# graphdeco-inria/hierarchical-3d-gaussians

Hardware: NVIDIA B200
Metric: train-step images/sec (fwd+bwd) @1080p, 3M Gaussians, SH-3 (higher is better)
Workload: dtype f32

## Files before the change

hierarchical-3d-gaussians_b200/csrc/common.cuh:

```cuda
#pragma once
#include <cuda_runtime.h>
#include <stdint.h>
#include <stdio.h>
#include <stdlib.h>
#include "../../include/h3dgs.h"

namespace h3dgs {

constexpr float kNearPlane = 0.2f;
constexpr float kFovClamp = 1.3f;
constexpr float kDilation = 0.3f;
constexpr float kLambdaFloor = 0.1f;
constexpr int kTile = H3DGS_TILE;
constexpr int kTilePixels = kTile * kTile;
constexpr float kAlphaCap = 0.99f;
constexpr float kAlphaSkip = 1.0f / 255.0f;
constexpr float kTStop = 0.0001f;
constexpr float kWEps = 0.0000001f;
constexpr uint32_t kKidsMask = 0xFFFFFu;
constexpr int kClampShift = 20;
constexpr uint32_t kSortedKidsMask = 0xFFFu;
constexpr int kBlockShift = 16;

struct __align__(16) Record { float4 a, b, c; };
static_assert(sizeof(Record) == 48, "record must be 48 bytes");

__host__ __device__ inline size_t align_up(size_t x, size_t a = 256) { return (x + a - 1) / a * a; }

struct GeomLayout {
    size_t depths, tiles_touched, offsets, rank_mask, records, scan_temp, total;
    size_t scan_temp_bytes;
};
struct BinLayout {
    size_t keys_unsorted, keys_sorted, vals_unsorted, vals_sorted, sort_temp, sorted_records, total;
    size_t sort_temp_bytes;
};
struct ImgLayout {
    size_t final_T, n_contrib, ranges, tile_max_contrib, tile_count, scan_info, total;
};
struct ScanInfo { uint32_t D, max_count, overflow, prefilter_bad; };
constexpr int kTileSortCap = 8192;

GeomLayout geom_layout(int P);
BinLayout bin_layout(int64_t D);
ImgLayout img_layout(int W, int H);

void prof_begin(int stage, cudaStream_t s);
void prof_end(int stage, cudaStream_t s);
struct ProfScope {
    int stage; cudaStream_t s;
    ProfScope(int st, cudaStream_t ss) : stage(st), s(ss) { prof_begin(stage, s); }
    ~ProfScope() { prof_end(stage, s); }
};

int pinned_scratch(void** out);

void set_error(const char* fmt, ...);
extern int64_t g_launches;

#define H3_CUDA(call)                                                                      \
    do {                                                                                   \
        cudaError_t e__ = (call);                                                          \
        if (e__ != cudaSuccess) {                                                          \
            h3dgs::set_error("%s failed at %s:%d: %s", #call, __FILE__, __LINE__,          \
                             cudaGetErrorString(e__));                                     \
            return H3DGS_ECUDA;                                                            \
        }                                                                                  \
    } while (0)

#define H3_LAUNCHED(name, debug, stream)                                                   \
    do {                                                                                   \
        h3dgs::g_launches++;                                                               \
        cudaError_t e__ = cudaGetLastError();                                              \
        if (e__ == cudaSuccess && (debug)) e__ = cudaStreamSynchronize(stream);            \
        if (e__ != cudaSuccess) {                                                          \
            h3dgs::set_error("kernel %s failed: %s", name, cudaGetErrorString(e__));       \
            return H3DGS_ECUDA;                                                            \
        }                                                                                  \
    } while (0)

int launch_preprocess(const h3dgs_raster_args& a, int32_t* radii, float* depths, uint32_t* tiles_touched,
                      uint8_t* rank_mask, Record* records, uint32_t* tile_count, ScanInfo* info, cudaStream_t s);
int launch_tile_scan(const h3dgs_raster_args& a, const uint32_t* tile_count, uint32_t* ranges, ScanInfo* info,
                     uint32_t cap_entries, uint32_t cap_list, cudaStream_t s);
int launch_tile_binning(const h3dgs_raster_args& a, const int32_t* radii, const float* depths, const Record* records,
                        int64_t D, uint32_t max_count, uint8_t* bin, const BinLayout& bl, const uint32_t* ranges,
                        const ScanInfo* info, uint32_t* tile_count, cudaStream_t s);
int launch_preprocess_color(const h3dgs_raster_args& a, const int32_t* radii, const uint32_t* tiles_touched,
                            Record* records, cudaStream_t s);
int launch_sh_backward(const h3dgs_raster_args& a, const int32_t* radii, const uint8_t* rank_mask, const Record* records,
                       const float* accum, float* dL_dmeans3D, float* dL_dsh, cudaStream_t s);
int launch_scan(const uint32_t* in, uint32_t* out, int n, void* temp, size_t temp_bytes, cudaStream_t s, bool debug);
size_t scan_temp_bytes(int n);
size_t sort_temp_bytes(int64_t n);
int launch_binning(const h3dgs_raster_args& a, const int32_t* radii, const float* depths, const uint32_t* offsets,
                   const Record* records, int64_t D, uint8_t* bin, const BinLayout& bl, uint32_t* ranges,
                   cudaStream_t s);
int launch_render_forward(const h3dgs_raster_args& a, const uint32_t* ranges, const Record* sorted_records,
                          float* out_color, float* out_invdepth, float* final_T, uint32_t* n_contrib,
                          uint32_t* tile_max_contrib, cudaStream_t s);
int launch_render_backward(const h3dgs_raster_args& a, const uint32_t* ranges, const Record* sorted_records,
                           const uint32_t* point_list, const float* final_T, const uint32_t* n_contrib,
                           const uint32_t* tile_max_contrib, const float* dL_dcolor, const float* dL_dinvdepth,
                           float* accum , cudaStream_t s);
int launch_preprocess_backward(const h3dgs_raster_args& a, const int32_t* radii, const uint8_t* rank_mask, const Record* records,
                               const float* accum, float* dL_dmeans3D, float* dL_dmeans2D, float* dL_dsh,
                               float* dL_dcolors, float* dL_dopacities, float* dL_dscales, float* dL_drots,
                               float* dL_dcov3D, cudaStream_t s);

#ifdef __CUDACC__
__device__ __forceinline__ void quad_pixel(int tile_x, int tile_y, int warp, int lane, int& px, int& py0) {
    px = tile_x * kTile + 8 * (warp & 1) + (lane & 7);
    py0 = tile_y * kTile + 8 * (warp >> 1) + 2 * (lane >> 3);
}

__device__ __forceinline__ void group_pixel(int tile_x, int tile_y, int warp, int lane, int& px, int& py0) {
    const int g = lane >> 3, k = lane & 7;
    px = tile_x * kTile + 8 * (warp & 1) + 4 * (g & 1) + (k & 3);
    py0 = tile_y * kTile + 8 * (warp >> 1) + 4 * (g >> 1) + 2 * (k >> 2);
}
inline bool use_group_walk() { const char* e = getenv("H3DGS_GROUPWALK"); return !(e && e[0] == '0'); }

#endif

struct PeerPtrs { void* p[H3DGS_MAX_PEERS]; int n; };
inline PeerPtrs peer_ptrs(void* const* src, int n) {
    PeerPtrs r; r.n = n > 1 ? n : 0;
    for (int k = 0; k < H3DGS_MAX_PEERS; k++) r.p[k] = (k < r.n) ? src[k] : nullptr;
    return r;
}
struct RowCycle { int shift, world, rank; };
inline RowCycle row_cycle(const h3dgs_raster_args& a) {
    RowCycle c; c.world = a.peer_count > 1 ? a.peer_count : 0; c.rank = a.shard_index; c.shift = a.grad_cyclic_log2;
    return c;
}
inline int cyclic_local_rows(const RowCycle& c, int P) {
    const int blocks = (P + (1 << c.shift) - 1) >> c.shift;
    return ((blocks + c.world - 1 - c.rank) / c.world) << c.shift;
}
#ifdef __CUDACC__
__device__ __forceinline__ int cyclic_row(const RowCycle& c, int local) {
    return ((((local >> c.shift) * c.world + c.rank)) << c.shift) + (local & ((1 << c.shift) - 1));
}
__device__ __forceinline__ bool cyclic_owned(const RowCycle& c, int row) { return ((row >> c.shift) % c.world) == c.rank; }
#endif

#ifdef __CUDACC__
struct StagePtrs { const float* own; const float* stage; int n, rank; size_t slot_floats; };
template <int NPAIR>
__device__ __forceinline__ void gather_accum_pairs(const StagePtrs& sp, uint32_t mask, int i, int first, float (&out)[2 * NPAIR]) {
#pragma unroll
    for (int k = 0; k < 2 * NPAIR; k++) out[k] = 0.f;
#pragma unroll
    for (int r = 0; r < H3DGS_MAX_PEERS; r++) {
        if (r < sp.n && ((mask >> r) & 1u)) {
            const float* row = (r == sp.rank ? sp.own : sp.stage + (size_t)r * sp.slot_floats) + (size_t)i * 10 + 2 * first;
#pragma unroll
            for (int k = 0; k < NPAIR; k++) {
                const float2 v = __ldcg(reinterpret_cast<const float2*>(row + 2 * k));
                out[2 * k] += v.x; out[2 * k + 1] += v.y;
            }
        }
    }
}
#endif
inline StagePtrs stage_ptrs(const h3dgs_raster_args& a, const float* accum) {
    StagePtrs sp; sp.own = accum; sp.n = a.peer_count > 1 ? a.peer_count : 0; sp.rank = a.shard_index;
    sp.stage = sp.n ? static_cast<const float*>(a.peer_stage[a.shard_index]) : nullptr;
    sp.slot_floats = (size_t)a.P * 10;
    return sp;
}
int launch_peer_push(const h3dgs_raster_args& a, const uint8_t* rank_mask, const float* accum, cudaStream_t s);

#ifdef H3_SIMT_EMU
extern long long g_emu_stats[16];
#define H3_STAT(i, n) (h3dgs::g_emu_stats[i] += (n))
#else
#define H3_STAT(i, n) ((void)0)
#endif

constexpr int kAccum = 10;

}

#ifdef __CUDACC__
#include "pair_math.cuh"
#endif
```

hierarchical-3d-gaussians_b200/csrc/pair_math.cuh:

```cuda
#pragma once

#ifdef H3_PAIR_HOST_EMU
#include <math.h>
#include <stdint.h>
#define H3_PM_FN static inline
namespace h3dgs {
#ifndef H3_SIMT_EMU
struct float4 { float x, y, z, w; };
constexpr float kAlphaCap = 0.99f;
constexpr float kAlphaSkip = 1.0f / 255.0f;
constexpr float kTStop = 0.0001f;
constexpr uint32_t kSortedKidsMask = 0xFFFu;
#endif
struct f2 { float lo, hi; };
H3_PM_FN f2 pk(float lo, float hi) { return f2{lo, hi}; }
H3_PM_FN void upk(f2 v, float& lo, float& hi) { lo = v.lo; hi = v.hi; }
H3_PM_FN f2 fma2(f2 a, f2 b, f2 c) { return f2{fmaf(a.lo, b.lo, c.lo), fmaf(a.hi, b.hi, c.hi)}; }
H3_PM_FN f2 mul2(f2 a, f2 b) { return f2{a.lo * b.lo, a.hi * b.hi}; }
H3_PM_FN f2 add2(f2 a, f2 b) { return f2{a.lo + b.lo, a.hi + b.hi}; }
H3_PM_FN f2 sub2(f2 a, f2 b) { return f2{a.lo - b.lo, a.hi - b.hi}; }
H3_PM_FN float fast_exp2(float x) { return exp2f(x); }
H3_PM_FN float fast_log2(float x) { return log2f(x); }
H3_PM_FN float rcp_approx(float x) { return 1.0f / x; }
H3_PM_FN float rsq_approx(float x) { return 1.0f / sqrtf(x); }
#else
#define H3_PM_FN __device__ __forceinline__
namespace h3dgs {
#ifdef H3_PAIR_SCALAR
struct f2 { float lo, hi; };
H3_PM_FN f2 pk(float lo, float hi) { return f2{lo, hi}; }
H3_PM_FN void upk(f2 v, float& lo, float& hi) { lo = v.lo; hi = v.hi; }
H3_PM_FN f2 fma2(f2 a, f2 b, f2 c) { return f2{__fmaf_rn(a.lo, b.lo, c.lo), __fmaf_rn(a.hi, b.hi, c.hi)}; }
H3_PM_FN f2 mul2(f2 a, f2 b) { return f2{__fmul_rn(a.lo, b.lo), __fmul_rn(a.hi, b.hi)}; }
H3_PM_FN f2 add2(f2 a, f2 b) { return f2{__fadd_rn(a.lo, b.lo), __fadd_rn(a.hi, b.hi)}; }
H3_PM_FN f2 sub2(f2 a, f2 b) { return f2{__fsub_rn(a.lo, b.lo), __fsub_rn(a.hi, b.hi)}; }
#else
typedef unsigned long long f2;
H3_PM_FN f2 pk(float lo, float hi) { f2 r; asm("mov.b64 %0, {%1, %2};" : "=l"(r) : "f"(lo), "f"(hi)); return r; }
H3_PM_FN void upk(f2 v, float& lo, float& hi) { asm("mov.b64 {%0, %1}, %2;" : "=f"(lo), "=f"(hi) : "l"(v)); }
H3_PM_FN f2 fma2(f2 a, f2 b, f2 c) { f2 d; asm("fma.rn.f32x2 %0, %1, %2, %3;" : "=l"(d) : "l"(a), "l"(b), "l"(c)); return d; }
H3_PM_FN f2 mul2(f2 a, f2 b) { f2 d; asm("mul.rn.f32x2 %0, %1, %2;" : "=l"(d) : "l"(a), "l"(b)); return d; }
H3_PM_FN f2 add2(f2 a, f2 b) { f2 d; asm("add.rn.f32x2 %0, %1, %2;" : "=l"(d) : "l"(a), "l"(b)); return d; }
H3_PM_FN f2 sub2(f2 a, f2 b) { f2 d; asm("sub.rn.f32x2 %0, %1, %2;" : "=l"(d) : "l"(a), "l"(b)); return d; }
#endif
H3_PM_FN float fast_exp2(float x) { float y; asm("ex2.approx.ftz.f32 %0, %1;" : "=f"(y) : "f"(x)); return y; }
H3_PM_FN float fast_log2(float x) { float y; asm("lg2.approx.ftz.f32 %0, %1;" : "=f"(y) : "f"(x)); return y; }
H3_PM_FN float rcp_approx(float x) { float y; asm("rcp.approx.ftz.f32 %0, %1;" : "=f"(y) : "f"(x)); return y; }
H3_PM_FN float rsq_approx(float x) { float y; asm("rsqrt.approx.ftz.f32 %0, %1;" : "=f"(y) : "f"(x)); return y; }
#endif

H3_PM_FN f2 bc(float x) { return pk(x, x); }
H3_PM_FN float lo(f2 v) { float a, b; upk(v, a, b); return a; }
H3_PM_FN float hi(f2 v) { float a, b; upk(v, a, b); return b; }
H3_PM_FN float hsum(f2 v) { float a, b; upk(v, a, b); return a + b; }
H3_PM_FN f2 sel2(bool p0, bool p1, f2 x, f2 y) {
    float x0, x1, y0, y1; upk(x, x0, x1); upk(y, y0, y1);
    return pk(p0 ? x0 : y0, p1 ? x1 : y1);
}
H3_PM_FN f2 ex2_2(f2 v) { float a, b; upk(v, a, b); return pk(fast_exp2(a), fast_exp2(b)); }
H3_PM_FN float fast_rcp(float x) { const float r = rcp_approx(x); return r * (2.0f - x * r); }
H3_PM_FN f2 rcp2(f2 x) {
    float x0, x1; upk(x, x0, x1);
    const f2 r = pk(rcp_approx(x0), rcp_approx(x1));
    return mul2(r, sub2(bc(2.0f), mul2(x, r)));
}

H3_PM_FN f2 pair_power(const float4& a, const float4& bb, float dx, f2 nfpy, f2& d) {
    d = add2(bc(a.y), nfpy);
    const float A = (a.z * dx) * (dx * -0.5f), B = -a.w * dx, C = -0.5f * bb.x;
    return fma2(fma2(bc(C), d, bc(B)), d, bc(A));
}
H3_PM_FN void pair_gauss(f2 power, float opacity, f2& G, f2& abase) {
    G = ex2_2(mul2(power, bc(1.4426950408889634f)));
    float a0, a1; upk(mul2(bc(opacity), G), a0, a1);
    abase = pk(fminf(kAlphaCap, a0), fminf(kAlphaCap, a1));
}
template <bool HIER, bool GRAD>
H3_PM_FN void pair_hier_alpha(f2 a, float t, uint32_t k , f2& alpha, f2& dadb) {
    alpha = a; dadb = bc(1.0f);
    if (!HIER) return;
    if (k <= 1u || t >= 1.0f) return;
    const float u = 1.0f - t;
    float a0, a1; upk(a, a0, a1);
    float o0, o1; upk(sub2(bc(1.0f), a), o0, o1);
    if (k == 2u) {
        const f2 r = pk(rsq_approx(o0), rsq_approx(o1));
        const f2 s = mul2(pk(o0, o1), r);
        f2 S = fma2(a, bc(0.02734375f), bc(0.0390625f));
        S = fma2(a, S, bc(0.0625f));
        S = fma2(a, S, bc(0.125f));
        S = fma2(a, S, bc(0.5f));
        const f2 omr = sel2(a0 < 0.0625f, a1 < 0.0625f, mul2(a, S), sub2(bc(1.0f), s));
        alpha = fma2(bc(u), omr, mul2(bc(t), a));
        if (GRAD) dadb = fma2(bc(0.5f * u), r, bc(t));
        return;
    }
    const float ik = fast_rcp((float)k);
    const f2 l2 = pk(fast_log2(o0), fast_log2(o1));
    f2 L = fma2(a, bc(0.2f), bc(0.25f));
    L = fma2(a, L, bc(0.33333334f));
    L = fma2(a, L, bc(0.5f));
    L = fma2(a, L, bc(1.0f));
    const f2 yn = mul2(mul2(a, L), bc(ik));
    f2 S = fma2(yn, bc(-0.041666668f), bc(0.16666667f));
    S = fma2(yn, S, bc(-0.5f));
    S = fma2(yn, S, bc(1.0f));
    const f2 omr_series = mul2(yn, S);
    const f2 omr_mufu = sub2(bc(1.0f), ex2_2(mul2(l2, bc(ik))));
    const f2 omr = sel2(a0 < 0.0625f, a1 < 0.0625f, omr_series, omr_mufu);
    alpha = fma2(bc(u), omr, mul2(bc(t), a));
    if (GRAD) dadb = fma2(bc(u * ik), ex2_2(mul2(l2, bc(ik - 1.0f))), bc(t));
}

H3_PM_FN f2 pair_blend(f2 pw, f2 al, f2& T, bool& done0, bool& done1, bool& v0, bool& v1, bool active = true) {
    const f2 tT = mul2(T, sub2(bc(1.0f), al));
    float pw0, pw1, al0, al1, tT0, tT1;
    upk(pw, pw0, pw1); upk(al, al0, al1); upk(tT, tT0, tT1);
    v0 = active && !done0 && pw0 <= 0.0f && al0 >= kAlphaSkip;
    v1 = active && !done1 && pw1 <= 0.0f && al1 >= kAlphaSkip;
    if (v0 && tT0 < kTStop) { done0 = true; v0 = false; }
    if (v1 && tT1 < kTStop) { done1 = true; v1 = false; }
    const f2 w = sel2(v0, v1, mul2(al, T), bc(0.f));
    T = sel2(v0, v1, tT, T);
    return w;
}

struct PairState { f2 T, acc; };

template <bool HIER, bool DEPTH>
H3_PM_FN void pair_grad(const float4& a, const float4& bb, float dx, f2 d, f2 G, f2 alpha, f2 dadb, f2 cg, f2 T_final,
                        f2 neg_bg_dot, f2 g0, f2 g1, f2 g2, f2 gd, PairState& st, float (&v)[10])
{
    const f2 rcp = rcp2(sub2(bc(1.0f), alpha));
    const f2 Tn = mul2(st.T, rcp);
    const f2 diff = sub2(cg, st.acc);
    const f2 dL_dalpha = fma2(mul2(T_final, rcp), neg_bg_dot, mul2(diff, Tn));
    const f2 dL_dab = HIER ? mul2(dL_dalpha, dadb) : dL_dalpha;
    const f2 w = mul2(alpha, Tn);
    st.T = Tn;
    st.acc = fma2(alpha, diff, st.acc);
    const f2 dL_dG = mul2(bc(bb.y), dL_dab);
    const f2 gdx = mul2(G, bc(dx)), gdy = mul2(G, d);
    const f2 qx = mul2(gdx, dL_dG), qy = mul2(gdy, dL_dG);
    v[0] = hsum(fma2(qy, bc(-a.w), mul2(qx, bc(-a.z))));
    v[1] = hsum(fma2(qx, bc(-a.w), mul2(qy, bc(-bb.x))));
    v[2] = hsum(qx) * dx;
    v[3] = hsum(mul2(qx, d));
    v[4] = hsum(mul2(qy, d));
    v[5] = hsum(mul2(G, dL_dab));
    v[6] = hsum(mul2(w, g0)); v[7] = hsum(mul2(w, g1)); v[8] = hsum(mul2(w, g2));
    v[9] = DEPTH ? hsum(mul2(w, gd)) : 0.f;
}

}
#undef H3_PM_FN
```

hierarchical-3d-gaussians_b200/csrc/render_backward.cu:

```cuda
#include "common.cuh"
#include "tma.cuh"

namespace h3dgs {

#ifdef H3_BLEND_OCC8
constexpr int kBwdBatch = 224;
constexpr int kBwdMinBlocks = 8;
#else
constexpr int kBwdBatch = 256;
constexpr int kBwdMinBlocks = 1;
#endif
constexpr int kBwdStages = 2;

__device__ __forceinline__ int reduce_slot(int lane) {
    if (lane & 1) return -1;
    const int b4 = (lane >> 4) & 1, b3 = (lane >> 3) & 1, b2 = (lane >> 2) & 1, b1 = (lane >> 1) & 1;
    int ai;
    if (!b3) { if (b2 && b1) return -1; ai = b2 ? 2 : b1; }
    else     { if (b2) return -1; ai = 3 + b1; }
    return 5 * b4 + ai;
}
__device__ __forceinline__ float xchg_add(float keep, float send, int mask) {
    return keep + __shfl_xor_sync(0xffffffffu, send, mask);
}
__device__ __forceinline__ f2 xchg_add2(float keep0, float send0, float keep1, float send1, int mask) {
    return add2(pk(keep0, keep1), pk(__shfl_xor_sync(0xffffffffu, send0, mask), __shfl_xor_sync(0xffffffffu, send1, mask)));
}
__device__ __forceinline__ float transpose_reduce10(const float (&v)[10], int lane) {
    const bool b4 = lane & 16, b3 = lane & 8, b2 = lane & 4, b1 = lane & 2;
    float a[5];
    upk(xchg_add2(b4 ? v[5] : v[0], b4 ? v[0] : v[5], b4 ? v[6] : v[1], b4 ? v[1] : v[6], 16), a[0], a[1]);
    upk(xchg_add2(b4 ? v[7] : v[2], b4 ? v[2] : v[7], b4 ? v[8] : v[3], b4 ? v[3] : v[8], 16), a[2], a[3]);
    a[4] = xchg_add(b4 ? v[9] : v[4], b4 ? v[4] : v[9], 16);
    float b[3];
    upk(xchg_add2(b3 ? a[3] : a[0], b3 ? a[0] : a[3], b3 ? a[4] : a[1], b3 ? a[1] : a[4], 8), b[0], b[1]);
    b[2] = xchg_add(b3 ? 0.f : a[2], b3 ? a[2] : 0.f, 8);
    float c[2];
    upk(xchg_add2(b2 ? b[2] : b[0], b2 ? b[0] : b[2], b2 ? 0.f : b[1], b2 ? b[1] : 0.f, 4), c[0], c[1]);
    float d = xchg_add(b1 ? c[1] : c[0], b1 ? c[0] : c[1], 2);
    d += __shfl_xor_sync(0xffffffffu, d, 1);
    return d;
}

__device__ __forceinline__ void group_slots(int k, int& s0, int& s1) {
    const int b2 = (k >> 2) & 1, b1 = (k >> 1) & 1, b0 = k & 1, base = 5 * b2;
    if (!b0) { s0 = base + (b1 ? 3 : 0); s1 = base + (b1 ? 4 : 1); }
    else { s0 = b1 ? -1 : base + 2; s1 = -1; }
}
__device__ __forceinline__ void transpose_reduce10_g8(const float (&v)[10], int lane, float& r0, float& r1) {
    const bool b2 = lane & 4, b1 = lane & 2, b0 = lane & 1;
    float a[5];
    upk(xchg_add2(b2 ? v[5] : v[0], b2 ? v[0] : v[5], b2 ? v[6] : v[1], b2 ? v[1] : v[6], 4), a[0], a[1]);
    upk(xchg_add2(b2 ? v[7] : v[2], b2 ? v[2] : v[7], b2 ? v[8] : v[3], b2 ? v[3] : v[8], 4), a[2], a[3]);
    a[4] = xchg_add(b2 ? v[9] : v[4], b2 ? v[4] : v[9], 4);
    float b[3];
    upk(xchg_add2(b1 ? a[3] : a[0], b1 ? a[0] : a[3], b1 ? a[4] : a[1], b1 ? a[1] : a[4], 2), b[0], b[1]);
    b[2] = xchg_add(b1 ? 0.f : a[2], b1 ? a[2] : 0.f, 2);
    upk(xchg_add2(b0 ? b[2] : b[0], b0 ? b[0] : b[2], b0 ? 0.f : b[1], b0 ? b[1] : 0.f, 1), r0, r1);
}

constexpr int kBwdThreads = 128;

template <bool HIER, bool DEPTH, bool GROUPS>
__global__ void __launch_bounds__(kBwdThreads, kBwdMinBlocks)
render_backward_kernel(int W, int H, int gx, int shard_count, int shard_index, const uint2* __restrict__ ranges,
                       const Record* __restrict__ sorted, const uint32_t* __restrict__ point_list,
                       const float* __restrict__ bg, const float* __restrict__ final_T,
                       const uint32_t* __restrict__ n_contrib, const uint32_t* __restrict__ tile_max_contrib,
                       const float* __restrict__ dL_dcolor, const float* __restrict__ dL_dinvdepth,
                       float* __restrict__ accum)
{
    __shared__ __align__(128) Record s_rec[kBwdStages][kBwdBatch];
    __shared__ uint32_t s_id[kBwdStages][kBwdBatch];
    __shared__ __align__(8) uint64_t s_full[kBwdStages];
    __shared__ uint8_t s_list[GROUPS ? kBwdThreads / 32 : 1][4][GROUPS ? kBwdBatch : 4];

    const int tid = threadIdx.x, lane = tid & 31, warp = tid >> 5;
    const int slot = reduce_slot(lane);
    const int tile_x = blockIdx.x % gx;
    const int tile_y = (blockIdx.x / gx) * shard_count + shard_index;
    const int tile = tile_y * gx + tile_x;
    const uint2 range = ranges[tile];
    const int n = min((int)(range.y - range.x), (int)tile_max_contrib[tile]);
    const int nb = (n + kBwdBatch - 1) / kBwdBatch;
    if (nb == 0) return;
    const Record* src = sorted + range.x;
    const uint32_t* ids = point_list + range.x;

    auto stage_ids = [&](int it) {
        const int b = nb - 1 - it, st = it % kBwdStages;
        for (int k = tid; k < kBwdBatch; k += kBwdThreads) {
            const int e = b * kBwdBatch + k;
            if (e < n) s_id[st][k] = ids[e];
        }
    };
    for (int it = 0; it < kBwdStages && it < nb; it++) stage_ids(it);
    if (tid == 0) {
        for (int s = 0; s < kBwdStages; s++) mbar_init(&s_full[s], 1);
        fence_mbar_init();
    }
    __syncthreads();
    auto issue = [&](int it) {
        const int b = nb - 1 - it, st = it % kBwdStages;
        const uint32_t bytes = (uint32_t)min(kBwdBatch, n - b * kBwdBatch) * (uint32_t)sizeof(Record);
        mbar_arrive_expect_tx(&s_full[st], bytes);
        tma_load_1d(&s_rec[st][0], src + (size_t)b * kBwdBatch, bytes, &s_full[st]);
    };
    if (tid == 0)
        for (int it = 0; it < kBwdStages && it < nb; it++) issue(it);

    int px, py0;
    if (GROUPS) group_pixel(tile_x, tile_y, warp, lane, px, py0);
    else quad_pixel(tile_x, tile_y, warp, lane, px, py0);
    int gs0, gs1;
    group_slots(lane & 7, gs0, gs1);
    const int grp = lane >> 3;
    const int py1 = py0 + 1;
    const bool in0 = px < W && py0 < H, in1 = px < W && py1 < H;
    const float fpx = (float)px;
    const f2 nfpy = pk(-(float)py0, -(float)py1);
    const size_t pix0 = (size_t)py0 * W + px, pix1 = (size_t)py1 * W + px, plane = (size_t)H * W;
    const float Tf0 = in0 ? final_T[pix0] : 0.f, Tf1 = in1 ? final_T[pix1] : 0.f;
    const f2 Tf = pk(Tf0, Tf1);
    PairState ps = {Tf, bc(0.f)};
    const int last0 = in0 ? (int)n_contrib[pix0] : 0, last1 = in1 ? (int)n_contrib[pix1] : 0;
    float ga0 = 0.f, ga1 = 0.f, ga2 = 0.f, gad = 0.f, gb0 = 0.f, gb1 = 0.f, gb2 = 0.f, gbd = 0.f;
    if (in0) { ga0 = dL_dcolor[pix0]; ga1 = dL_dcolor[plane + pix0]; ga2 = dL_dcolor[2 * plane + pix0]; if (DEPTH) gad = dL_dinvdepth[pix0]; }
    if (in1) { gb0 = dL_dcolor[pix1]; gb1 = dL_dcolor[plane + pix1]; gb2 = dL_dcolor[2 * plane + pix1]; if (DEPTH) gbd = dL_dinvdepth[pix1]; }
    const f2 g0 = pk(ga0, gb0), g1 = pk(ga1, gb1), g2 = pk(ga2, gb2), gd = pk(gad, gbd);
    const f2 neg_bgd = pk(-(bg[0] * ga0 + bg[1] * ga1 + bg[2] * ga2), -(bg[0] * gb0 + bg[1] * gb1 + bg[2] * gb2));
    const int wlast = (int)__reduce_max_sync(0xffffffffu, (unsigned)max(last0, last1));
    const int qsel = kBlockShift + 4 * warp;
    int gl0, gl1, gl2, gl3;
    {
        int gm = max(last0, last1);
        gm = max(gm, __shfl_xor_sync(0xffffffffu, gm, 4)); gm = max(gm, __shfl_xor_sync(0xffffffffu, gm, 2));
        gm = max(gm, __shfl_xor_sync(0xffffffffu, gm, 1));
        gl0 = __shfl_sync(0xffffffffu, gm, 0); gl1 = __shfl_sync(0xffffffffu, gm, 8);
        gl2 = __shfl_sync(0xffffffffu, gm, 16); gl3 = __shfl_sync(0xffffffffu, gm, 24);
    }

    for (int it = 0; it < nb; it++) {
        const int st = it % kBwdStages, b = nb - 1 - it;
        mbar_wait(&s_full[st], (uint32_t)((it / kBwdStages) & 1));
        const int cnt = min(kBwdBatch, n - b * kBwdBatch);
        const Record* rec = &s_rec[st][0];
        auto replay_entry = [&](int j, bool has) {
            const int e = b * kBwdBatch + j;
            const float4 a = rec[j].a;
            const float4 bb = rec[j].b;
            const uint32_t gid = s_id[st][j];
            const uint32_t kb = __float_as_uint(bb.w);
            const float dx = a.x - fpx;
            f2 d, G, al, dadb = bc(1.0f);
            const f2 pw = pair_power(a, bb, dx, nfpy, d);
            pair_gauss(pw, bb.y, G, al);
            float pw0, pw1, al0, al1;
            upk(pw, pw0, pw1); upk(al, al0, al1);
            bool v0 = has && e < last0 && pw0 <= 0.0f && al0 >= kAlphaSkip;
            bool v1 = has && e < last1 && pw1 <= 0.0f && al1 >= kAlphaSkip;
            if (lane == 0) H3_STAT(0, 1);
            if ((lane & 7) == 0 && has) H3_STAT(3, 1);
            if (!__any_sync(0xffffffffu, v0 || v1)) { if (lane == 0) H3_STAT(1, 1); return; }
            if (HIER) {
                pair_hier_alpha<HIER, true>(al, bb.z, kb & kSortedKidsMask, al, dadb);
                upk(al, al0, al1);
                v0 = v0 && al0 >= kAlphaSkip;
                v1 = v1 && al1 >= kAlphaSkip;
            }
            H3_STAT(2, (v0 ? 1 : 0) + (v1 ? 1 : 0));
#ifdef H3_SIMT_EMU
            { const uint32_t tk = __ballot_sync(0xffffffffu, v0 || v1);
              if (GROUPS && (lane & 7) == 0 && has && ((tk >> (8 * grp)) & 0xFFu) == 0u) H3_STAT(4, 1); }
#endif
            G = sel2(v0, v1, G, bc(0.f));
            al = sel2(v0, v1, al, bc(0.f));
            const float4 c = rec[j].c;
            f2 cg = fma2(bc(c.z), g2, fma2(bc(c.y), g1, mul2(bc(c.x), g0)));
            if (DEPTH) cg = fma2(bc(c.w), gd, cg);
            float v[10];
            pair_grad<HIER, DEPTH>(a, bb, dx, d, G, al, dadb, cg, Tf, neg_bgd, g0, g1, g2, gd, ps, v);
            if (GROUPS) {
                const bool taker = ((__ballot_sync(0xffffffffu, v0 || v1) >> (8 * grp)) & 0xFFu) != 0u;
                float r0, r1;
                transpose_reduce10_g8(v, lane, r0, r1);
                float* row = accum + (size_t)gid * kAccum;
                if (taker && gs0 >= 0 && (DEPTH || gs0 < 9)) atomicAdd(row + gs0, r0);
                if (taker && gs1 >= 0 && (DEPTH || gs1 < 9)) atomicAdd(row + gs1, r1);
            } else {
                const float total = transpose_reduce10(v, lane);
                float* row = accum + (size_t)gid * kAccum;
                if (slot >= 0 && (DEPTH || slot < 9)) atomicAdd(row + slot, total);
            }
        };
        if (GROUPS) {
            uint8_t* lst = &s_list[warp][0][0];
            const uint32_t lt = (1u << lane) - 1u;
            int c0 = 0, c1 = 0, c2 = 0, c3 = 0;
            for (int j0 = 0; j0 < cnt; j0 += 32) {
                const int jl = j0 + lane, e = b * kBwdBatch + jl;
                uint32_t nib = jl < cnt ? (__float_as_uint(rec[jl].b.w) >> qsel) & 0xFu : 0u;
                nib &= (e < gl0 ? 1u : 0u) | (e < gl1 ? 2u : 0u) | (e < gl2 ? 4u : 0u) | (e < gl3 ? 8u : 0u);
                const uint32_t m0 = __ballot_sync(0xffffffffu, nib & 1u), m1 = __ballot_sync(0xffffffffu, nib & 2u);
                const uint32_t m2 = __ballot_sync(0xffffffffu, nib & 4u), m3 = __ballot_sync(0xffffffffu, nib & 8u);
                if (nib & 1u) lst[c0 + __popc(m0 & lt)] = (uint8_t)jl;
                if (nib & 2u) lst[kBwdBatch + c1 + __popc(m1 & lt)] = (uint8_t)jl;
                if (nib & 4u) lst[2 * kBwdBatch + c2 + __popc(m2 & lt)] = (uint8_t)jl;
                if (nib & 8u) lst[3 * kBwdBatch + c3 + __popc(m3 & lt)] = (uint8_t)jl;
                c0 += __popc(m0); c1 += __popc(m1); c2 += __popc(m2); c3 += __popc(m3);
            }
            __syncwarp();
            const int mylen = grp == 0 ? c0 : grp == 1 ? c1 : grp == 2 ? c2 : c3;
            const int maxlen = max(max(c0, c1), max(c2, c3));
            const uint8_t* my = lst + grp * kBwdBatch;
            for (int i = maxlen - 1; i >= 0; i--) {
                const bool has = i < mylen;
                replay_entry(has ? (int)my[i] : 0, has);
            }
            __syncwarp();
        } else {
            for (int j0 = (cnt - 1) & ~31; j0 >= 0; j0 -= 32) {
                const int jl = j0 + lane;
                const uint32_t nib = (jl < cnt && (b * kBwdBatch + jl) < wlast) ? (__float_as_uint(rec[jl].b.w) >> qsel) & 0xFu : 0u;
                uint32_t m = __ballot_sync(0xffffffffu, nib != 0u);
                while (m != 0u) {
                    const int top = 31 - __clz(m);
                    m &= ~(1u << top);
                    replay_entry(j0 + top, true);
                }
            }
        }
        __syncthreads();
        if (it + kBwdStages < nb) {
            if (tid == 0) issue(it + kBwdStages);
            stage_ids(it + kBwdStages);
        }
    }
}

int launch_render_backward(const h3dgs_raster_args& a, const uint32_t* ranges, const Record* sorted_records,
                           const uint32_t* point_list, const float* final_T, const uint32_t* n_contrib,
                           const uint32_t* tile_max_contrib, const float* dL_dcolor, const float* dL_dinvdepth,
                           float* accum, cudaStream_t s)
{
    const int W = a.image_width, H = a.image_height;
    const int gx = (W + kTile - 1) / kTile, gy = (H + kTile - 1) / kTile;
    const int sc = a.shard_count > 0 ? a.shard_count : 1, si = a.shard_count > 0 ? a.shard_index : 0;
    const int rows = (gy + sc - 1 - si) / sc;
    if (rows <= 0 || gx <= 0) return H3DGS_OK;
    const bool hier = a.interpolation_weights != nullptr;
    const bool depth = a.do_depth != 0 && dL_dinvdepth != nullptr;
    const dim3 grid(gx * rows), block(kBwdThreads);
    ProfScope prof(H3DGS_STAGE_RENDER_BWD, s);
    const bool groups = use_group_walk();
#define LAUNCH(HI, DE, GR)                                                                                          \
    render_backward_kernel<HI, DE, GR><<<grid, block, 0, s>>>(W, H, gx, sc, si, (const uint2*)ranges, sorted_records, \
                                                              point_list, a.bg, final_T, n_contrib, tile_max_contrib, \
                                                              dL_dcolor, dL_dinvdepth, accum)
#define LAUNCH2(HI, DE) do { if (groups) LAUNCH(HI, DE, true); else LAUNCH(HI, DE, false); } while (0)
    if (hier) { if (depth) LAUNCH2(true, true); else LAUNCH2(true, false); }
    else      { if (depth) LAUNCH2(false, true); else LAUNCH2(false, false); }
#undef LAUNCH2
#undef LAUNCH
    H3_LAUNCHED("render_backward", a.debug, s);
    return H3DGS_OK;
}

}
```

Before: 521.2.

## Remap group-walk backward to 64-thread blocks with four pixels per thread

The group-walk render backward kernel now runs 64 threads per block, each thread covering four pixels as two vertical pairs. Groups of four lanes cover 4x4 pixel blocks, with eight groups per warp using an 8-bit per-warp mask. Per-Gaussian gradient terms are summed across both pairs in registers before a shorter 4-lane transpose-reduce, which cuts shuffles and atomics per pixel. The batch shrinks to 128 and the kernel asks for 10 resident blocks per SM. In exchange, register pressure rises, the list-building work per warp grows, and the qsel bit layout assumes 8 bits per warp in the record mask.

```diff
diff --git a/hierarchical-3d-gaussians_b200/csrc/common.cuh b/hierarchical-3d-gaussians_b200/csrc/common.cuh
--- a/hierarchical-3d-gaussians_b200/csrc/common.cuh
+++ b/hierarchical-3d-gaussians_b200/csrc/common.cuh
@@ -119,6 +119,11 @@
     px = tile_x * kTile + 8 * (warp & 1) + 4 * (g & 1) + (k & 3);
     py0 = tile_y * kTile + 8 * (warp >> 1) + 4 * (g >> 1) + 2 * (k >> 2);
 }
+__device__ __forceinline__ void block_pixel(int tile_x, int tile_y, int warp, int lane, int& px, int& py0) {
+    const int g = lane >> 2, k = lane & 3;
+    px = tile_x * kTile + 8 * (g >> 2) + 4 * (g & 1) + k;
+    py0 = tile_y * kTile + 8 * warp + 4 * ((g >> 1) & 1);
+}
 inline bool use_group_walk() { const char* e = getenv("H3DGS_GROUPWALK"); return !(e && e[0] == '0'); }
 
 #endif
diff --git a/hierarchical-3d-gaussians_b200/csrc/pair_math.cuh b/hierarchical-3d-gaussians_b200/csrc/pair_math.cuh
--- a/hierarchical-3d-gaussians_b200/csrc/pair_math.cuh
+++ b/hierarchical-3d-gaussians_b200/csrc/pair_math.cuh
@@ -128,8 +128,8 @@
 struct PairState { f2 T, acc; };
 
 template <bool HIER, bool DEPTH>
-H3_PM_FN void pair_grad(const float4& a, const float4& bb, float dx, f2 d, f2 G, f2 alpha, f2 dadb, f2 cg, f2 T_final,
-                        f2 neg_bg_dot, f2 g0, f2 g1, f2 g2, f2 gd, PairState& st, float (&v)[10])
+H3_PM_FN void pair_grad_terms(const float4& a, const float4& bb, float dx, f2 d, f2 G, f2 alpha, f2 dadb, f2 cg,
+                              f2 T_final, f2 neg_bg_dot, f2 g0, f2 g1, f2 g2, f2 gd, PairState& st, f2 (&t)[10])
 {
     const f2 rcp = rcp2(sub2(bc(1.0f), alpha));
     const f2 Tn = mul2(st.T, rcp);
@@ -142,14 +142,25 @@
     const f2 dL_dG = mul2(bc(bb.y), dL_dab);
     const f2 gdx = mul2(G, bc(dx)), gdy = mul2(G, d);
     const f2 qx = mul2(gdx, dL_dG), qy = mul2(gdy, dL_dG);
-    v[0] = hsum(fma2(qy, bc(-a.w), mul2(qx, bc(-a.z))));
-    v[1] = hsum(fma2(qx, bc(-a.w), mul2(qy, bc(-bb.x))));
-    v[2] = hsum(qx) * dx;
-    v[3] = hsum(mul2(qx, d));
-    v[4] = hsum(mul2(qy, d));
-    v[5] = hsum(mul2(G, dL_dab));
-    v[6] = hsum(mul2(w, g0)); v[7] = hsum(mul2(w, g1)); v[8] = hsum(mul2(w, g2));
-    v[9] = DEPTH ? hsum(mul2(w, gd)) : 0.f;
+    t[0] = fma2(qy, bc(-a.w), mul2(qx, bc(-a.z)));
+    t[1] = fma2(qx, bc(-a.w), mul2(qy, bc(-bb.x)));
+    t[2] = qx;
+    t[3] = mul2(qx, d);
+    t[4] = mul2(qy, d);
+    t[5] = mul2(G, dL_dab);
+    t[6] = mul2(w, g0); t[7] = mul2(w, g1); t[8] = mul2(w, g2);
+    t[9] = DEPTH ? mul2(w, gd) : bc(0.f);
+}
+
+template <bool HIER, bool DEPTH>
+H3_PM_FN void pair_grad(const float4& a, const float4& bb, float dx, f2 d, f2 G, f2 alpha, f2 dadb, f2 cg, f2 T_final,
+                        f2 neg_bg_dot, f2 g0, f2 g1, f2 g2, f2 gd, PairState& st, float (&v)[10])
+{
+    f2 t[10];
+    pair_grad_terms<HIER, DEPTH>(a, bb, dx, d, G, alpha, dadb, cg, T_final, neg_bg_dot, g0, g1, g2, gd, st, t);
+#pragma unroll
+    for (int k = 0; k < 10; k++) v[k] = hsum(t[k]);
+    v[2] *= dx;
 }
 
 }
diff --git a/hierarchical-3d-gaussians_b200/csrc/render_backward.cu b/hierarchical-3d-gaussians_b200/csrc/render_backward.cu
--- a/hierarchical-3d-gaussians_b200/csrc/render_backward.cu
+++ b/hierarchical-3d-gaussians_b200/csrc/render_backward.cu
@@ -3,13 +3,11 @@
 
 namespace h3dgs {
 
-#ifdef H3_BLEND_OCC8
-constexpr int kBwdBatch = 224;
-constexpr int kBwdMinBlocks = 8;
-#else
+constexpr int kBwdThreads = 128;
 constexpr int kBwdBatch = 256;
-constexpr int kBwdMinBlocks = 1;
-#endif
+constexpr int kBwdGroupThreads = 64;
+constexpr int kBwdGroupBatch = 128;
+constexpr int kBwdGroupMinBlocks = 10;
 constexpr int kBwdStages = 2;
 
 __device__ __forceinline__ int reduce_slot(int lane) {
@@ -42,27 +40,23 @@
     return d;
 }
 
-__device__ __forceinline__ void group_slots(int k, int& s0, int& s1) {
-    const int b2 = (k >> 2) & 1, b1 = (k >> 1) & 1, b0 = k & 1, base = 5 * b2;
-    if (!b0) { s0 = base + (b1 ? 3 : 0); s1 = base + (b1 ? 4 : 1); }
-    else { s0 = b1 ? -1 : base + 2; s1 = -1; }
-}
-__device__ __forceinline__ void transpose_reduce10_g8(const float (&v)[10], int lane, float& r0, float& r1) {
-    const bool b2 = lane & 4, b1 = lane & 2, b0 = lane & 1;
+__device__ __forceinline__ void group4_slots(int k, int& s0, int& s1, int& s2) {
+    const int base = 5 * ((k >> 1) & 1);
+    if (!(k & 1)) { s0 = base; s1 = base + 1; s2 = base + 2; }
+    else { s0 = base + 3; s1 = base + 4; s2 = -1; }
+}
+__device__ __forceinline__ void transpose_reduce10_g4(const float (&v)[10], int lane, float& r0, float& r1, float& r2) {
+    const bool b1 = lane & 2, b0 = lane & 1;
     float a[5];
-    upk(xchg_add2(b2 ? v[5] : v[0], b2 ? v[0] : v[5], b2 ? v[6] : v[1], b2 ? v[1] : v[6], 4), a[0], a[1]);
-    upk(xchg_add2(b2 ? v[7] : v[2], b2 ? v[2] : v[7], b2 ? v[8] : v[3], b2 ? v[3] : v[8], 4), a[2], a[3]);
-    a[4] = xchg_add(b2 ? v[9] : v[4], b2 ? v[4] : v[9], 4);
-    float b[3];
-    upk(xchg_add2(b1 ? a[3] : a[0], b1 ? a[0] : a[3], b1 ? a[4] : a[1], b1 ? a[1] : a[4], 2), b[0], b[1]);
-    b[2] = xchg_add(b1 ? 0.f : a[2], b1 ? a[2] : 0.f, 2);
-    upk(xchg_add2(b0 ? b[2] : b[0], b0 ? b[0] : b[2], b0 ? 0.f : b[1], b0 ? b[1] : 0.f, 1), r0, r1);
-}
-
-constexpr int kBwdThreads = 128;
+    upk(xchg_add2(b1 ? v[5] : v[0], b1 ? v[0] : v[5], b1 ? v[6] : v[1], b1 ? v[1] : v[6], 2), a[0], a[1]);
+    upk(xchg_add2(b1 ? v[7] : v[2], b1 ? v[2] : v[7], b1 ? v[8] : v[3], b1 ? v[3] : v[8], 2), a[2], a[3]);
+    a[4] = xchg_add(b1 ? v[9] : v[4], b1 ? v[4] : v[9], 2);
+    upk(xchg_add2(b0 ? a[3] : a[0], b0 ? a[0] : a[3], b0 ? a[4] : a[1], b0 ? a[1] : a[4], 1), r0, r1);
+    r2 = xchg_add(b0 ? 0.f : a[2], b0 ? a[2] : 0.f, 1);
+}
 
 template <bool HIER, bool DEPTH, bool GROUPS>
-__global__ void __launch_bounds__(kBwdThreads, kBwdMinBlocks)
+__global__ void __launch_bounds__(GROUPS ? kBwdGroupThreads : kBwdThreads, GROUPS ? kBwdGroupMinBlocks : 1)
 render_backward_kernel(int W, int H, int gx, int shard_count, int shard_index, const uint2* __restrict__ ranges,
                        const Record* __restrict__ sorted, const uint32_t* __restrict__ point_list,
                        const float* __restrict__ bg, const float* __restrict__ final_T,
@@ -70,10 +64,13 @@
                        const float* __restrict__ dL_dcolor, const float* __restrict__ dL_dinvdepth,
                        float* __restrict__ accum)
 {
-    __shared__ __align__(128) Record s_rec[kBwdStages][kBwdBatch];
-    __shared__ uint32_t s_id[kBwdStages][kBwdBatch];
+    constexpr int NT = GROUPS ? kBwdGroupThreads : kBwdThreads;
+    constexpr int BATCH = GROUPS ? kBwdGroupBatch : kBwdBatch;
+    constexpr int NP = GROUPS ? 2 : 1;
+    __shared__ __align__(128) Record s_rec[kBwdStages][BATCH];
+    __shared__ uint32_t s_id[kBwdStages][BATCH];
     __shared__ __align__(8) uint64_t s_full[kBwdStages];
-    __shared__ uint8_t s_list[GROUPS ? kBwdThreads / 32 : 1][4][GROUPS ? kBwdBatch : 4];
+    __shared__ uint8_t s_list[GROUPS ? NT / 32 : 1][GROUPS ? 8 : 1][GROUPS ? BATCH : 4];
 
     const int tid = threadIdx.x, lane = tid & 31, warp = tid >> 5;
     const int slot = reduce_slot(lane);
@@ -82,15 +79,15 @@
     const int tile = tile_y * gx + tile_x;
     const uint2 range = ranges[tile];
     const int n = min((int)(range.y - range.x), (int)tile_max_contrib[tile]);
-    const int nb = (n + kBwdBatch - 1) / kBwdBatch;
+    const int nb = (n + BATCH - 1) / BATCH;
     if (nb == 0) return;
     const Record* src = sorted + range.x;
     const uint32_t* ids = point_list + range.x;
 
     auto stage_ids = [&](int it) {
         const int b = nb - 1 - it, st = it % kBwdStages;
-        for (int k = tid; k < kBwdBatch; k += kBwdThreads) {
-            const int e = b * kBwdBatch + k;
+        for (int k = tid; k < BATCH; k += NT) {
+            const int e = b * BATCH + k;
             if (e < n) s_id[st][k] = ids[e];
         }
     };
@@ -102,117 +99,159 @@
     __syncthreads();
     auto issue = [&](int it) {
         const int b = nb - 1 - it, st = it % kBwdStages;
-        const uint32_t bytes = (uint32_t)min(kBwdBatch, n - b * kBwdBatch) * (uint32_t)sizeof(Record);
+        const uint32_t bytes = (uint32_t)min(BATCH, n - b * BATCH) * (uint32_t)sizeof(Record);
         mbar_arrive_expect_tx(&s_full[st], bytes);
-        tma_load_1d(&s_rec[st][0], src + (size_t)b * kBwdBatch, bytes, &s_full[st]);
+        tma_load_1d(&s_rec[st][0], src + (size_t)b * BATCH, bytes, &s_full[st]);
     };
     if (tid == 0)
         for (int it = 0; it < kBwdStages && it < nb; it++) issue(it);
 
     int px, py0;
-    if (GROUPS) group_pixel(tile_x, tile_y, warp, lane, px, py0);
+    if (GROUPS) block_pixel(tile_x, tile_y, warp, lane, px, py0);
     else quad_pixel(tile_x, tile_y, warp, lane, px, py0);
-    int gs0, gs1;
-    group_slots(lane & 7, gs0, gs1);
-    const int grp = lane >> 3;
-    const int py1 = py0 + 1;
-    const bool in0 = px < W && py0 < H, in1 = px < W && py1 < H;
+    int gs0, gs1, gs2;
+    group4_slots(lane & 3, gs0, gs1, gs2);
+    const int grp = lane >> 2;
     const float fpx = (float)px;
-    const f2 nfpy = pk(-(float)py0, -(float)py1);
-    const size_t pix0 = (size_t)py0 * W + px, pix1 = (size_t)py1 * W + px, plane = (size_t)H * W;
-    const float Tf0 = in0 ? final_T[pix0] : 0.f, Tf1 = in1 ? final_T[pix1] : 0.f;
-    const f2 Tf = pk(Tf0, Tf1);
-    PairState ps = {Tf, bc(0.f)};
-    const int last0 = in0 ? (int)n_contrib[pix0] : 0, last1 = in1 ? (int)n_contrib[pix1] : 0;
-    float ga0 = 0.f, ga1 = 0.f, ga2 = 0.f, gad = 0.f, gb0 = 0.f, gb1 = 0.f, gb2 = 0.f, gbd = 0.f;
-    if (in0) { ga0 = dL_dcolor[pix0]; ga1 = dL_dcolor[plane + pix0]; ga2 = dL_dcolor[2 * plane + pix0]; if (DEPTH) gad = dL_dinvdepth[pix0]; }
-    if (in1) { gb0 = dL_dcolor[pix1]; gb1 = dL_dcolor[plane + pix1]; gb2 = dL_dcolor[2 * plane + pix1]; if (DEPTH) gbd = dL_dinvdepth[pix1]; }
-    const f2 g0 = pk(ga0, gb0), g1 = pk(ga1, gb1), g2 = pk(ga2, gb2), gd = pk(gad, gbd);
-    const f2 neg_bgd = pk(-(bg[0] * ga0 + bg[1] * ga1 + bg[2] * ga2), -(bg[0] * gb0 + bg[1] * gb1 + bg[2] * gb2));
-    const int wlast = (int)__reduce_max_sync(0xffffffffu, (unsigned)max(last0, last1));
-    const int qsel = kBlockShift + 4 * warp;
-    int gl0, gl1, gl2, gl3;
+    const size_t plane = (size_t)H * W;
+    f2 nfpy[NP], Tf[NP], g0[NP], g1[NP], g2[NP], gd[NP], neg_bgd[NP];
+    PairState ps[NP];
+    int last[2 * NP];
+    int tlast = 0;
+#pragma unroll
+    for (int p = 0; p < NP; p++) {
+        float T[2] = {0.f, 0.f}, c0[2] = {0.f, 0.f}, c1[2] = {0.f, 0.f}, c2[2] = {0.f, 0.f}, cd[2] = {0.f, 0.f};
+#pragma unroll
+        for (int r = 0; r < 2; r++) {
+            const int py = py0 + 2 * p + r;
+            const size_t pix = (size_t)py * W + px;
+            last[2 * p + r] = 0;
+            if (px < W && py < H) {
+                T[r] = final_T[pix];
+                last[2 * p + r] = (int)n_contrib[pix];
+                c0[r] = dL_dcolor[pix]; c1[r] = dL_dcolor[plane + pix]; c2[r] = dL_dcolor[2 * plane + pix];
+                if (DEPTH) cd[r] = dL_dinvdepth[pix];
+            }
+            tlast = max(tlast, last[2 * p + r]);
+        }
+        nfpy[p] = pk(-(float)(py0 + 2 * p), -(float)(py0 + 2 * p + 1));
+        Tf[p] = pk(T[0], T[1]);
+        ps[p] = {Tf[p], bc(0.f)};
+        g0[p] = pk(c0[0], c0[1]); g1[p] = pk(c1[0], c1[1]); g2[p] = pk(c2[0], c2[1]); gd[p] = pk(cd[0], cd[1]);
+        neg_bgd[p] = pk(-(bg[0] * c0[0] + bg[1] * c1[0] + bg[2] * c2[0]), -(bg[0] * c0[1] + bg[1] * c1[1] + bg[2] * c2[1]));
+    }
+    const int wlast = (int)__reduce_max_sync(0xffffffffu, (unsigned)tlast);
+    const int qsel = kBlockShift + (GROUPS ? 8 : 4) * warp;
+    int gl[8];
     {
-        int gm = max(last0, last1);
-        gm = max(gm, __shfl_xor_sync(0xffffffffu, gm, 4)); gm = max(gm, __shfl_xor_sync(0xffffffffu, gm, 2));
+        int gm = max(tlast, __shfl_xor_sync(0xffffffffu, tlast, 2));
         gm = max(gm, __shfl_xor_sync(0xffffffffu, gm, 1));
-        gl0 = __shfl_sync(0xffffffffu, gm, 0); gl1 = __shfl_sync(0xffffffffu, gm, 8);
-        gl2 = __shfl_sync(0xffffffffu, gm, 16); gl3 = __shfl_sync(0xffffffffu, gm, 24);
+#pragma unroll
+        for (int g = 0; g < 8; g++) gl[g] = __shfl_sync(0xffffffffu, gm, 4 * g);
     }
 
     for (int it = 0; it < nb; it++) {
         const int st = it % kBwdStages, b = nb - 1 - it;
         mbar_wait(&s_full[st], (uint32_t)((it / kBwdStages) & 1));
-        const int cnt = min(kBwdBatch, n - b * kBwdBatch);
+        const int cnt = min(BATCH, n - b * BATCH);
         const Record* rec = &s_rec[st][0];
         auto replay_entry = [&](int j, bool has) {
-            const int e = b * kBwdBatch + j;
+            const int e = b * BATCH + j;
             const float4 a = rec[j].a;
             const float4 bb = rec[j].b;
             const uint32_t gid = s_id[st][j];
             const uint32_t kb = __float_as_uint(bb.w);
             const float dx = a.x - fpx;
-            f2 d, G, al, dadb = bc(1.0f);
-            const f2 pw = pair_power(a, bb, dx, nfpy, d);
-            pair_gauss(pw, bb.y, G, al);
-            float pw0, pw1, al0, al1;
-            upk(pw, pw0, pw1); upk(al, al0, al1);
-            bool v0 = has && e < last0 && pw0 <= 0.0f && al0 >= kAlphaSkip;
-            bool v1 = has && e < last1 && pw1 <= 0.0f && al1 >= kAlphaSkip;
+            f2 d[NP], G[NP], al[NP], dadb[NP];
+            bool v[2 * NP], any = false;
+#pragma unroll
+            for (int p = 0; p < NP; p++) {
+                const f2 pw = pair_power(a, bb, dx, nfpy[p], d[p]);
+                pair_gauss(pw, bb.y, G[p], al[p]);
+                dadb[p] = bc(1.0f);
+                float pw0, pw1, al0, al1;
+                upk(pw, pw0, pw1); upk(al[p], al0, al1);
+                v[2 * p] = has && e < last[2 * p] && pw0 <= 0.0f && al0 >= kAlphaSkip;
+                v[2 * p + 1] = has && e < last[2 * p + 1] && pw1 <= 0.0f && al1 >= kAlphaSkip;
+                any = any || v[2 * p] || v[2 * p + 1];
+            }
             if (lane == 0) H3_STAT(0, 1);
-            if ((lane & 7) == 0 && has) H3_STAT(3, 1);
-            if (!__any_sync(0xffffffffu, v0 || v1)) { if (lane == 0) H3_STAT(1, 1); return; }
+            if (GROUPS && (lane & 3) == 0 && has) H3_STAT(3, 1);
+            if (!__any_sync(0xffffffffu, any)) { if (lane == 0) H3_STAT(1, 1); return; }
             if (HIER) {
-                pair_hier_alpha<HIER, true>(al, bb.z, kb & kSortedKidsMask, al, dadb);
-                upk(al, al0, al1);
-                v0 = v0 && al0 >= kAlphaSkip;
-                v1 = v1 && al1 >= kAlphaSkip;
-            }
-            H3_STAT(2, (v0 ? 1 : 0) + (v1 ? 1 : 0));
+                any = false;
+#pragma unroll
+                for (int p = 0; p < NP; p++) {
+                    pair_hier_alpha<HIER, true>(al[p], bb.z, kb & kSortedKidsMask, al[p], dadb[p]);
+                    float al0, al1;
+                    upk(al[p], al0, al1);
+                    v[2 * p] = v[2 * p] && al0 >= kAlphaSkip;
+                    v[2 * p + 1] = v[2 * p + 1] && al1 >= kAlphaSkip;
+                    any = any || v[2 * p] || v[2 * p + 1];
+                }
+            }
 #ifdef H3_SIMT_EMU
-            { const uint32_t tk = __ballot_sync(0xffffffffu, v0 || v1);
-              if (GROUPS && (lane & 7) == 0 && has && ((tk >> (8 * grp)) & 0xFFu) == 0u) H3_STAT(4, 1); }
+#pragma unroll
+            for (int p = 0; p < NP; p++) H3_STAT(2, (v[2 * p] ? 1 : 0) + (v[2 * p + 1] ? 1 : 0));
+            { const uint32_t tk = __ballot_sync(0xffffffffu, any);
+              if (GROUPS && (lane & 3) == 0 && has && ((tk >> (4 * grp)) & 0xFu) == 0u) H3_STAT(4, 1); }
 #endif
-            G = sel2(v0, v1, G, bc(0.f));
-            al = sel2(v0, v1, al, bc(0.f));
             const float4 c = rec[j].c;
-            f2 cg = fma2(bc(c.z), g2, fma2(bc(c.y), g1, mul2(bc(c.x), g0)));
-            if (DEPTH) cg = fma2(bc(c.w), gd, cg);
-            float v[10];
-            pair_grad<HIER, DEPTH>(a, bb, dx, d, G, al, dadb, cg, Tf, neg_bgd, g0, g1, g2, gd, ps, v);
+            f2 t[10];
+#pragma unroll
+            for (int p = 0; p < NP; p++) {
+                G[p] = sel2(v[2 * p], v[2 * p + 1], G[p], bc(0.f));
+                al[p] = sel2(v[2 * p], v[2 * p + 1], al[p], bc(0.f));
+                f2 cg = fma2(bc(c.z), g2[p], fma2(bc(c.y), g1[p], mul2(bc(c.x), g0[p])));
+                if (DEPTH) cg = fma2(bc(c.w), gd[p], cg);
+                f2 tp[10];
+                pair_grad_terms<HIER, DEPTH>(a, bb, dx, d[p], G[p], al[p], dadb[p], cg, Tf[p], neg_bgd[p], g0[p], g1[p], g2[p],
+                                             gd[p], ps[p], tp);
+#pragma unroll
+                for (int k = 0; k < 10; k++) t[k] = p == 0 ? tp[k] : add2(t[k], tp[k]);
+            }
+            float vs[10];
+#pragma unroll
+            for (int k = 0; k < 10; k++) vs[k] = hsum(t[k]);
+            vs[2] *= dx;
+            float* row = accum + (size_t)gid * kAccum;
             if (GROUPS) {
-                const bool taker = ((__ballot_sync(0xffffffffu, v0 || v1) >> (8 * grp)) & 0xFFu) != 0u;
-                float r0, r1;
-                transpose_reduce10_g8(v, lane, r0, r1);
-                float* row = accum + (size_t)gid * kAccum;
-                if (taker && gs0 >= 0 && (DEPTH || gs0 < 9)) atomicAdd(row + gs0, r0);
-                if (taker && gs1 >= 0 && (DEPTH || gs1 < 9)) atomicAdd(row + gs1, r1);
+                const bool taker = ((__ballot_sync(0xffffffffu, any) >> (4 * grp)) & 0xFu) != 0u;
+                float r0, r1, r2;
+                transpose_reduce10_g4(vs, lane, r0, r1, r2);
+                if (taker && (DEPTH || gs0 < 9)) atomicAdd(row + gs0, r0);
+                if (taker && (DEPTH || gs1 < 9)) atomicAdd(row + gs1, r1);
+                if (taker && gs2 >= 0) atomicAdd(row + gs2, r2);
             } else {
-                const float total = transpose_reduce10(v, lane);
-                float* row = accum + (size_t)gid * kAccum;
+                const float total = transpose_reduce10(vs, lane);
                 if (slot >= 0 && (DEPTH || slot < 9)) atomicAdd(row + slot, total);
             }
         };
         if (GROUPS) {
             uint8_t* lst = &s_list[warp][0][0];
             const uint32_t lt = (1u << lane) - 1u;
-            int c0 = 0, c1 = 0, c2 = 0, c3 = 0;
+            int c[8];
+#pragma unroll
+            for (int g = 0; g < 8; g++) c[g] = 0;
             for (int j0 = 0; j0 < cnt; j0 += 32) {
-                const int jl = j0 + lane, e = b * kBwdBatch + jl;
-                uint32_t nib = jl < cnt ? (__float_as_uint(rec[jl].b.w) >> qsel) & 0xFu : 0u;
-                nib &= (e < gl0 ? 1u : 0u) | (e < gl1 ? 2u : 0u) | (e < gl2 ? 4u : 0u) | (e < gl3 ? 8u : 0u);
-                const uint32_t m0 = __ballot_sync(0xffffffffu, nib & 1u), m1 = __ballot_sync(0xffffffffu, nib & 2u);
-                const uint32_t m2 = __ballot_sync(0xffffffffu, nib & 4u), m3 = __ballot_sync(0xffffffffu, nib & 8u);
-                if (nib & 1u) lst[c0 + __popc(m0 & lt)] = (uint8_t)jl;
-                if (nib & 2u) lst[kBwdBatch + c1 + __popc(m1 & lt)] = (uint8_t)jl;
-                if (nib & 4u) lst[2 * kBwdBatch + c2 + __popc(m2 & lt)] = (uint8_t)jl;
-                if (nib & 8u) lst[3 * kBwdBatch + c3 + __popc(m3 & lt)] = (uint8_t)jl;
-                c0 += __popc(m0); c1 += __popc(m1); c2 += __popc(m2); c3 += __popc(m3);
+                const int jl = j0 + lane, e = b * BATCH + jl;
+                uint32_t byte = jl < cnt ? (__float_as_uint(rec[jl].b.w) >> qsel) & 0xFFu : 0u;
+                uint32_t live = 0u;
+#pragma unroll
+                for (int g = 0; g < 8; g++) live |= (e < gl[g] ? 1u : 0u) << g;
+                byte &= live;
+#pragma unroll
+                for (int g = 0; g < 8; g++) {
+                    const uint32_t m = __ballot_sync(0xffffffffu, (byte >> g) & 1u);
+                    if ((byte >> g) & 1u) lst[g * BATCH + c[g] + __popc(m & lt)] = (uint8_t)jl;
+                    c[g] += __popc(m);
+                }
             }
             __syncwarp();
-            const int mylen = grp == 0 ? c0 : grp == 1 ? c1 : grp == 2 ? c2 : c3;
-            const int maxlen = max(max(c0, c1), max(c2, c3));
-            const uint8_t* my = lst + grp * kBwdBatch;
+            int mylen = 0, maxlen = 0;
+#pragma unroll
+            for (int g = 0; g < 8; g++) { mylen = g == grp ? c[g] : mylen; maxlen = max(maxlen, c[g]); }
+            const uint8_t* my = lst + grp * BATCH;
             for (int i = maxlen - 1; i >= 0; i--) {
                 const bool has = i < mylen;
                 replay_entry(has ? (int)my[i] : 0, has);
@@ -221,7 +260,7 @@
         } else {
             for (int j0 = (cnt - 1) & ~31; j0 >= 0; j0 -= 32) {
                 const int jl = j0 + lane;
-                const uint32_t nib = (jl < cnt && (b * kBwdBatch + jl) < wlast) ? (__float_as_uint(rec[jl].b.w) >> qsel) & 0xFu : 0u;
+                const uint32_t nib = (jl < cnt && (b * BATCH + jl) < wlast) ? (__float_as_uint(rec[jl].b.w) >> qsel) & 0xFu : 0u;
                 uint32_t m = __ballot_sync(0xffffffffu, nib != 0u);
                 while (m != 0u) {
                     const int top = 31 - __clz(m);
@@ -250,9 +289,10 @@
     if (rows <= 0 || gx <= 0) return H3DGS_OK;
     const bool hier = a.interpolation_weights != nullptr;
     const bool depth = a.do_depth != 0 && dL_dinvdepth != nullptr;
-    const dim3 grid(gx * rows), block(kBwdThreads);
+    const dim3 grid(gx * rows);
     ProfScope prof(H3DGS_STAGE_RENDER_BWD, s);
     const bool groups = use_group_walk();
+    const dim3 block(groups ? kBwdGroupThreads : kBwdThreads);
 #define LAUNCH(HI, DE, GR)                                                                                          \
     render_backward_kernel<HI, DE, GR><<<grid, block, 0, s>>>(W, H, gx, sc, si, (const uint2*)ranges, sorted_records, \
                                                               point_list, a.bg, final_T, n_contrib, tile_max_contrib, \
```

After: 520.3, median of 6. Within noise of the previous version (-0.2%).
